# davidesantangelo/krep

Measured on NVIDIA H100. Metric: GB/s scanned (HBM-resident corpus), higher is better.
Workload: dtype u8

## Files before the change

krep_b200/csrc/common.h:

```cpp
#pragma once
#include <cuda_runtime.h>
#include <stdint.h>
#include <stddef.h>
#include <string>
#include <vector>
#include "../../include/krep_b200.h"

namespace kb {

static constexpr int LIT_TAG_BITS = 3;
static constexpr int AC_END_SHIFT = 24;
static constexpr int AC_LEN_SHIFT = 14;
static constexpr uint32_t AC_MAX_PATTERNS = 1u << 14;

enum FilterKind : int
{
    FILTER_ALIGNED4 = 0,
    FILTER_WINDOW4 = 1,
};

struct LitDevParams
{
    const uint8_t *text;
    uint64_t avail_len;
    uint64_t own_begin, own_end;
    uint64_t global_offset;
    int32_t prev_byte, next_byte;
    uint64_t group_begin, group_end;
    uint64_t tail_start;
    uint32_t m;
    uint32_t emit_len;
    uint32_t K[4];
    uint32_t fold;
    uint32_t win_mask;
    uint32_t mulc[3];
    const uint8_t *pat_val;
    const uint8_t *pat_mask;
    uint64_t *out;
    uint64_t cap;
    unsigned long long *counter;
    uint32_t whole_word;
    uint32_t want_positions;
};

struct AcDevTables;
struct AcHostTables;

static constexpr int MAX_DEV = 16;

struct PlanDev
{
    bool ready = false;
    uint8_t *d_pat_val = nullptr, *d_pat_mask = nullptr;
    AcDevTables *ac = nullptr;
};

struct Plan
{
    int algo = 0;
    bool is_ac = false;
    std::string pattern;
    bool case_sensitive = true;
    uint32_t m = 0, emit_len = 0;
    FilterKind filter = FILTER_ALIGNED4;
    uint32_t K[4] = {0, 0, 0, 0};
    uint32_t fold = 0xFFFFFFFFu, win_mask = 0xFFFFFFFFu;
    uint32_t whole_word = 0;
    std::vector<uint8_t> h_val, h_msk;
    bool border_free = true;
    bool built_only_matching = false;
    bool count_lines = false;
    std::vector<std::string> patterns;
    std::vector<uint32_t> pat_lens;
    uint32_t min_len = 0, max_len = 0;
    AcHostTables *ach = nullptr;
    std::string filter_name;
    PlanDev dev[MAX_DEV];
    uint64_t magic = 0x6b7265705f623230ull;
};

struct DevCtx;
void set_error(int code, const char *fmt, ...);
void clear_error();

struct ScanOut
{
    uint64_t count = 0, stored = 0;
    const uint64_t *d_keys = nullptr;
    int overflow = 0;
    const uint64_t *d_bounds = nullptr;
    const uint64_t *h_sorted = nullptr;
    int device = 0;
    uint64_t serial = 0;
};

static constexpr uint64_t LB_SAME_AS_PREV = ~0ull;
static constexpr uint64_t LB_SAME_AS_NEXT = ~0ull - 1;
static constexpr uint64_t LB_OUTSIDE_SHARD = ~0ull - 2;

int launch_scan(DevCtx &C, const Plan *plan, const krep_b200_shard_t *sh, int want_positions, cudaStream_t stream, int slot = 0);
void launch_literal(const Plan *plan, const LitDevParams &p, int sm_count, cudaStream_t s);
int ac_build_tables(Plan *plan);
void ac_free_tables(Plan *plan);
AcDevTables *ac_upload_tables(const Plan *plan);
void ac_free_device(AcDevTables *T);
struct AcLaunch
{
    const uint8_t *text;
    uint64_t avail_len, own_begin, own_end, global_offset;
    int32_t prev_byte, next_byte;
    uint64_t *out;
    uint64_t cap;
    unsigned long long *counter;
    uint32_t whole_word, want_positions;
};
void launch_ac(const Plan *plan, const AcDevTables *T, const AcLaunch &a, int sm_count, cudaStream_t s);
void count_launch(int n = 1);

struct Replay
{
    const uint64_t *keys;
    size_t n;
    const char *text;
    size_t text_len;
    uint64_t base;
    const uint64_t *bounds = nullptr;
};
uint64_t replay_literal(int algo, const search_params_t *P, bool only_matching, uint32_t m,
                        const Replay &r, match_result_t *res);
uint64_t replay_ac(const search_params_t *P, const Replay &r, match_result_t *res);
bool result_push(match_result_t *r, size_t s, size_t e);

static inline unsigned char lower_c(unsigned char c) { return (c >= 'A' && c <= 'Z') ? (unsigned char)(c + 32) : c; }
static inline bool is_alpha_c(unsigned char c) { return (c >= 'A' && c <= 'Z') || (c >= 'a' && c <= 'z'); }
static inline bool is_word_c(int c)
{
    return (c >= '0' && c <= '9') || (c >= 'A' && c <= 'Z') || (c >= 'a' && c <= 'z') || c == '_';
}

}
```

krep_b200/csrc/engine.cu:

```cuda
#include <cub/device/device_radix_sort.cuh>
#include <algorithm>
#include <chrono>
#include <cstdarg>
#include <cstdio>
#include <cstdlib>
#include <cstring>
#include <mutex>
#include <thread>
#include "common.h"
#include "corpus.h"
#include "engine.h"

namespace kb {

static thread_local int t_err = 0;
static thread_local char t_errmsg[512] = "";

void set_error(int code, const char *fmt, ...)
{
    t_err = code;
    va_list ap;
    va_start(ap, fmt);
    vsnprintf(t_errmsg, sizeof t_errmsg, fmt, ap);
    va_end(ap);
    fprintf(stderr, "krep: %s\n", t_errmsg);
}
void clear_error()
{
    t_err = 0;
    t_errmsg[0] = 0;
}

#define CK(call)                                                                                   \
    do                                                                                             \
    {                                                                                              \
        cudaError_t e_ = (call);                                                                   \
        if (e_ != cudaSuccess)                                                                     \
        {                                                                                          \
            set_error(-2, "CUDA error %s at %s:%d (%s)", cudaGetErrorName(e_), __FILE__, __LINE__, \
                      cudaGetErrorString(e_));                                                     \
            return -2;                                                                             \
        }                                                                                          \
    } while (0)

static DevCtx g_ctx[MAX_DEV];
static std::recursive_mutex g_mu;
static std::mutex g_ctx_mu;
static int g_primary = -1;
static int g_visible = -1;
static bool g_keep_visible = false;
static uint64_t g_launches = 0;
static thread_local float t_kernel_ms = 0.f;
static const std::chrono::steady_clock::time_point g_t0 = std::chrono::steady_clock::now();

std::recursive_mutex &engine_mutex() { return g_mu; }
void count_launch(int n) { __atomic_fetch_add(&g_launches, (uint64_t)n, __ATOMIC_RELAXED); }
void add_kernel_ms(float ms) { t_kernel_ms += ms; }
void reset_kernel_ms() { t_kernel_ms = 0.f; }
float get_kernel_ms() { return t_kernel_ms; }
void set_kernel_ms(float ms) { t_kernel_ms = ms; }
void get_error(ErrState *e)
{
    e->code = t_err;
    memcpy(e->msg, t_errmsg, sizeof e->msg);
}
void adopt_error(const ErrState &e)
{
    t_err = e.code;
    memcpy(t_errmsg, e.msg, sizeof t_errmsg);
}

void trace(const char *fmt, ...)
{
    static const bool on = getenv("KREP_B200_TRACE") != nullptr;
    if (!on) return;
    char buf[400];
    va_list ap;
    va_start(ap, fmt);
    vsnprintf(buf, sizeof buf, fmt, ap);
    va_end(ap);
    const double ms = std::chrono::duration<double, std::milli>(std::chrono::steady_clock::now() - g_t0).count();
    fprintf(stderr, "[krep_b200 +%.1f ms] %s\n", ms, buf);
}

static std::thread *g_warm = nullptr;
static std::mutex g_warm_mu;
void warm_join()
{
    std::lock_guard<std::mutex> lk(g_warm_mu);
    if (g_warm && g_warm->joinable() && g_warm->get_id() != std::this_thread::get_id()) g_warm->join();
}
bool warm_running()
{
    std::lock_guard<std::mutex> lk(g_warm_mu);
    return g_warm && g_warm->joinable();
}
static void warm_start()
{
    std::lock_guard<std::mutex> lk(g_warm_mu);
    if (g_warm || g_visible >= 0) return;
    g_warm = new std::thread([] {
        trace("warm-up thread: start");
        if (visible_devices() > 0)
            if (DevCtx *C = ctx_primary()) prewarm_host_path(*C);
        trace("warm-up thread: done");
    });
}
__attribute__((destructor)) static void warm_at_exit()
{
    warm_join();
    trace("library destructor (process exit)");
}

void keep_devices_visible() { g_keep_visible = true; }

int visible_devices()
{
    if (g_visible >= 0) return g_visible;
    static std::mutex mu;
    std::lock_guard<std::mutex> lk(mu);
    if (g_visible >= 0) return g_visible;
    if (!g_keep_visible && !getenv("KREP_B200_KEEP_VISIBLE"))
    {
        const char *v = getenv("KREP_B200_DEVICES");
        const int k = v && atoi(v) > 0 ? atoi(v) : 1;
        std::string list;
        if (const char *cur = getenv("CUDA_VISIBLE_DEVICES"))
        {
            int taken = 0;
            for (const char *q = cur; *q && taken < k;)
            {
                const char *e = strchr(q, ',');
                const size_t len = e ? (size_t)(e - q) : strlen(q);
                if (len)
                {
                    list += (taken ? "," : "") + std::string(q, len);
                    taken++;
                }
                q += len + (e ? 1 : 0);
            }
        }
        else
            for (int d = 0; d < k && d < MAX_DEV; d++) list += (d ? "," : "") + std::to_string(d);
        if (!list.empty())
        {
            setenv("CUDA_VISIBLE_DEVICES", list.c_str(), 1);
            trace("CUDA_VISIBLE_DEVICES=%s", list.c_str());
        }
    }
    int n = 0;
    trace("cudaGetDeviceCount ...");
    cudaError_t e = cudaGetDeviceCount(&n);
    if (e != cudaSuccess)
    {
        cudaGetLastError();
        n = 0;
    }
    trace("cudaGetDeviceCount -> %d", n);
    g_visible = n > MAX_DEV ? MAX_DEV : n;
    return g_visible;
}

int primary_device()
{
    if (g_primary >= 0) return g_primary;
    if (visible_devices() == 0)
    {
        set_error(-1, "no CUDA device available; this engine has no CPU fallback");
        return -1;
    }
    int d = 0;
    if (cudaGetDevice(&d) != cudaSuccess) d = 0;
    g_primary = d;
    return d;
}

static int ctx_create(DevCtx &E, int device)
{
    trace("device %d: creating context", device);
    CK(cudaSetDevice(device));
    cudaDeviceProp prop;
    CK(cudaGetDeviceProperties(&prop, device));
    if (prop.major != 9 || prop.minor != 0)
    {
        set_error(-1, "device %d (%s, sm_%d%d) is not an sm_90 part; kernels are built for sm_90a only", device,
                  prop.name, prop.major, prop.minor);
        return -1;
    }
    E.device = device;
    E.sm_count = prop.multiProcessorCount;
    CK(cudaStreamCreateWithFlags(&E.scan_stream, cudaStreamNonBlocking));
    CK(cudaStreamCreateWithFlags(&E.copy_stream, cudaStreamNonBlocking));
    CK(cudaStreamCreateWithFlags(&E.fin_stream, cudaStreamNonBlocking));
    CK(cudaMalloc(&E.d_counter, 64 * SCAN_SLOTS));
    CK(cudaMemset(E.d_counter, 0, 64 * SCAN_SLOTS));
    CK(cudaEventCreate(&E.ev_ca));
    CK(cudaEventCreate(&E.ev_cb));
    for (int s = 0; s < SCAN_SLOTS; s++)
    {
        CK(cudaMalloc(&E.d_pack[s], (PACK_KEYS + 1) * sizeof(uint64_t)));
        CK(cudaHostAlloc(&E.h_pack[s], (PACK_KEYS + 1) * sizeof(uint64_t), cudaHostAllocMapped | cudaHostAllocPortable));
        E.h_pack[s][0] = 0;
        CK(cudaEventCreate(&E.ev_a[s]));
        CK(cudaEventCreate(&E.ev_b[s]));
        CK(cudaEventCreateWithFlags(&E.ev_done[s], cudaEventDisableTiming));
        CK(cudaEventCreateWithFlags(&E.ev_scanned[s], cudaEventDisableTiming));
        E.counter_clean[s] = true;
    }
    E.ready = true;
    trace("device %d: context ready (%s, %d SMs)", device, prop.name, E.sm_count);
    return 0;
}

DevCtx *ctx_get(int device)
{
    if (device < 0 || device >= MAX_DEV || device >= visible_devices())
    {
        set_error(-1, visible_devices() == 0 ? "no CUDA device available; this engine has no CPU fallback"
                                               : "CUDA device %d is not visible to this process",
                  device);
        return nullptr;
    }
    DevCtx &E = g_ctx[device];
    if (E.ready)
    {
        cudaSetDevice(device);
        return &E;
    }
    static std::mutex mu[MAX_DEV];
    std::lock_guard<std::mutex> lk(mu[device]);
    if (!E.ready && ctx_create(E, device) != 0) return nullptr;
    return &E;
}

DevCtx *ctx_primary()
{
    const int d = primary_device();
    return d < 0 ? nullptr : ctx_get(d);
}

static std::vector<Plan *> g_all_plans;
static std::mutex g_plans_mu;

static void ctx_destroy(DevCtx &E)
{
    if (!E.ready) return;
    cudaSetDevice(E.device);
    cudaDeviceSynchronize();
    for (int s = 0; s < SCAN_SLOTS; s++) cudaFree(E.d_list[s]);
    cudaFree(E.d_alt);
    cudaFree(E.d_sort_tmp);
    cudaFree(E.d_bounds);
    cudaFreeHost(E.h_bounds);
    cudaFreeHost(E.h_batch);
    cudaFree(E.d_counter);
    cudaFree(E.d_ring);
    cudaFree(E.d_line_recs);
    cudaFree(E.d_line_out);
    cudaFreeHost(E.h_line_out);
    cudaFreeHost(E.h_keys);
    for (int s = 0; s < SCAN_SLOTS; s++)
    {
        cudaFree(E.d_pack[s]);
        cudaFreeHost(E.h_pack[s]);
        cudaEventDestroy(E.ev_a[s]);
        cudaEventDestroy(E.ev_b[s]);
        cudaEventDestroy(E.ev_done[s]);
        cudaEventDestroy(E.ev_scanned[s]);
    }
    for (auto &s : E.stage) cudaFreeHost(s.buf);
    for (auto &s : E.stage)
        if (s.ev) cudaEventDestroy(s.ev);
    for (auto ev : E.ev_pool) cudaEventDestroy(ev);
    for (auto ev : E.ring_landed) cudaEventDestroy(ev);
    for (auto ev : E.ring_scanned) cudaEventDestroy(ev);
    cudaEventDestroy(E.ev_ca);
    cudaEventDestroy(E.ev_cb);
    cudaStreamDestroy(E.scan_stream);
    cudaStreamDestroy(E.copy_stream);
    cudaStreamDestroy(E.fin_stream);
    E = DevCtx();
}

void plan_cache_clear();

void engine_shutdown()
{
    std::lock_guard<std::recursive_mutex> lk(g_mu);
    DeviceGuard guard;
    plan_cache_clear();
    {
        std::lock_guard<std::mutex> lp(g_plans_mu);
        for (Plan *p : g_all_plans)
            for (int d = 0; d < MAX_DEV; d++)
            {
                PlanDev &pd = p->dev[d];
                if (!pd.ready) continue;
                cudaSetDevice(d);
                cudaFree(pd.d_pat_val);
                cudaFree(pd.d_pat_mask);
                if (pd.ac) ac_free_device(pd.ac);
                pd = PlanDev();
            }
    }
    for (int d = 0; d < MAX_DEV; d++) ctx_destroy(g_ctx[d]);
    g_primary = -1;
}

int ensure_keys(DevCtx &E, uint64_t cap)
{
    if (cap <= E.key_cap) return 0;
    uint64_t ncap = E.key_cap ? E.key_cap : (1ull << 20);
    while (ncap < cap) ncap *= 2;
    CK(cudaDeviceSynchronize());
    for (int s = 0; s < SCAN_SLOTS; s++)
    {
        cudaFree(E.d_list[s]);
        E.d_list[s] = nullptr;
    }
    cudaFree(E.d_alt);
    E.d_alt = nullptr;
    E.key_cap = 0;
    for (int s = 0; s < SCAN_SLOTS; s++) CK(cudaMalloc(&E.d_list[s], ncap * sizeof(uint64_t)));
    CK(cudaMalloc(&E.d_alt, ncap * sizeof(uint64_t)));
    E.key_cap = ncap;
    return 0;
}

unsigned long long *slot_counter(DevCtx &E, int slot) { return E.d_counter + 8 * slot; }

static uint32_t le32(const uint8_t *b, uint32_t n)
{
    uint32_t v = 0;
    for (uint32_t k = 0; k < n && k < 4; k++) v |= (uint32_t)b[k] << (8 * k);
    return v;
}

void plan_free(Plan *p)
{
    if (!p) return;
    {
        std::lock_guard<std::mutex> lp(g_plans_mu);
        for (size_t i = 0; i < g_all_plans.size(); i++)
            if (g_all_plans[i] == p)
            {
                g_all_plans.erase(g_all_plans.begin() + i);
                break;
            }
    }
    DeviceGuard guard;
    for (int d = 0; d < MAX_DEV; d++)
    {
        PlanDev &pd = p->dev[d];
        if (!pd.ready) continue;
        cudaSetDevice(d);
        cudaFree(pd.d_pat_val);
        cudaFree(pd.d_pat_mask);
        if (pd.ac) ac_free_device(pd.ac);
    }
    if (p->ach) ac_free_tables(p);
    p->magic = 0;
    delete p;
}

const PlanDev *plan_on_device(const Plan *plan, DevCtx &C)
{
    static std::mutex mu;
    PlanDev &pd = const_cast<Plan *>(plan)->dev[C.device];
    if (pd.ready) return &pd;
    std::lock_guard<std::mutex> lk(mu);
    if (pd.ready) return &pd;
    cudaSetDevice(C.device);
    if (plan->is_ac)
    {
        pd.ac = ac_upload_tables(plan);
        if (!pd.ac) return nullptr;
    }
    else
    {
        const size_t m = plan->h_val.size();
        if (cudaMalloc(&pd.d_pat_val, m) != cudaSuccess || cudaMalloc(&pd.d_pat_mask, m) != cudaSuccess ||
            cudaMemcpy(pd.d_pat_val, plan->h_val.data(), m, cudaMemcpyHostToDevice) != cudaSuccess ||
            cudaMemcpy(pd.d_pat_mask, plan->h_msk.data(), m, cudaMemcpyHostToDevice) != cudaSuccess)
        {
            set_error(-2, "CUDA allocation failed while uploading the pattern to device %d", C.device);
            cudaFree(pd.d_pat_val);
            cudaFree(pd.d_pat_mask);
            pd = PlanDev();
            return nullptr;
        }
    }
    pd.ready = true;
    return &pd;
}

static bool border_free(const std::string &s, bool cs)
{
    const size_t m = s.size();
    if (m < 2) return true;
    std::vector<int> pi(m, 0);
    auto ch = [&](size_t i) { return cs ? (unsigned char)s[i] : lower_c((unsigned char)s[i]); };
    for (size_t i = 1; i < m; i++)
    {
        int k = pi[i - 1];
        while (k > 0 && ch(i) != ch((size_t)k)) k = pi[(size_t)k - 1];
        if (ch(i) == ch((size_t)k)) k++;
        pi[i] = k;
    }
    return pi[m - 1] == 0;
}

Plan *plan_build(const search_params_t *P, int algo, bool only_matching)
{
    if (!P) return nullptr;
    Plan *pl = new Plan();
    pl->algo = algo;
    pl->case_sensitive = P->case_sensitive;
    pl->count_lines = P->count_lines_mode;
    if (algo == KREP_B200_ALGO_AC)
    {
        pl->is_ac = true;
        if (P->num_patterns > AC_MAX_PATTERNS)
        {
            set_error(-3, "too many patterns (%zu > %u)", (size_t)P->num_patterns, AC_MAX_PATTERNS);
            delete pl;
            return nullptr;
        }
        for (size_t k = 0; k < P->num_patterns; k++)
        {
            const size_t len = P->pattern_lens[k];
            if (len > 1024)
            {
                set_error(-3, "pattern %zu longer than 1024 bytes (krep.c:77)", k);
                delete pl;
                return nullptr;
            }
            pl->patterns.emplace_back(P->patterns[k] ? P->patterns[k] : "", len);
            pl->pat_lens.push_back((uint32_t)len);
        }
        pl->whole_word = P->whole_word ? 1 : 0;
        if (ac_build_tables(pl) != 0)
        {
            delete pl;
            return nullptr;
        }
        std::lock_guard<std::mutex> lp(g_plans_mu);
        g_all_plans.push_back(pl);
        return pl;
    }
    size_t m = P->pattern_len;
    if (algo == KREP_B200_ALGO_MEMCHR) m = m ? 1 : 0;
    if (m == 0 || m > 1024 || !P->pattern)
    {
        set_error(-3, "literal plan needs 1..1024 pattern bytes (got %zu)", m);
        delete pl;
        return nullptr;
    }
    pl->pattern.assign(P->pattern, m);
    pl->m = (uint32_t)m;
    pl->emit_len = (algo == KREP_B200_ALGO_MEMCHR_SHORT && only_matching) ? 1u : (uint32_t)m;
    pl->border_free = border_free(pl->pattern, pl->case_sensitive);
    pl->built_only_matching = only_matching;
    if (P->whole_word)
    {
        bool tag = pl->emit_len != pl->m;
        if (algo == KREP_B200_ALGO_AVX2 || algo == KREP_B200_ALGO_AVX512 || algo == KREP_B200_ALGO_NEON) tag = true;
        if (!tag && !pl->border_free)
            tag = algo == KREP_B200_ALGO_KMP || (algo == KREP_B200_ALGO_SSE42 && !only_matching);
        pl->whole_word = tag ? 2 : 1;
    }
    pl->h_val.resize(m);
    pl->h_msk.resize(m);
    const uint8_t *pb = (const uint8_t *)pl->pattern.data();
    for (size_t k = 0; k < m; k++)
    {
        pl->h_msk[k] = (!pl->case_sensitive && is_alpha_c(pb[k])) ? 0xDF : 0xFF;
        pl->h_val[k] = pb[k] & pl->h_msk[k];
    }
    pl->fold = pl->case_sensitive ? 0xFFFFFFFFu : 0xDFDFDFDFu;
    if (pl->emit_len >= 7)
    {
        pl->filter = FILTER_ALIGNED4;
        for (int d = 0; d < 4; d++) pl->K[d] = le32(pb + d, 4) & pl->fold;
        pl->win_mask = 0xFFFFFFFFu;
        pl->filter_name = pl->case_sensitive ? "aligned4" : "aligned4-fold";
    }
    else
    {
        pl->filter = FILTER_WINDOW4;
        const uint32_t wl = pl->emit_len < 4 ? pl->emit_len : 4;
        pl->win_mask = wl == 4 ? 0xFFFFFFFFu : ((1u << (8 * wl)) - 1);
        pl->K[0] = le32(pb, wl) & pl->fold & pl->win_mask;
        pl->filter_name = pl->case_sensitive ? "window4" : "window4-fold";
    }
    std::lock_guard<std::mutex> lp(g_plans_mu);
    g_all_plans.push_back(pl);
    return pl;
}

int launch_scan(DevCtx &E, const Plan *plan, const krep_b200_shard_t *sh, int want_positions, cudaStream_t stream, int slot)
{
    if (((uintptr_t)sh->d_text & 15) != 0)
    {
        set_error(-3, "shard text pointer must be 16-byte aligned");
        return -3;
    }
    const PlanDev *pd = plan_on_device(plan, E);
    if (!pd) return -2;
    uint64_t own_end = sh->own_end < sh->avail_len ? sh->own_end : sh->avail_len;
    if (plan->is_ac)
    {
        if (sh->global_offset + sh->avail_len >= (1ull << 40))
        {
            set_error(-3, "pattern-set shards must end below 2^40 bytes of global offset (key layout, csrc/common.h)");
            return -3;
        }
        AcLaunch a;
        a.text = (const uint8_t *)sh->d_text;
        a.avail_len = sh->avail_len;
        a.own_begin = sh->own_begin;
        a.own_end = own_end;
        a.global_offset = sh->global_offset;
        a.prev_byte = sh->prev_byte;
        a.next_byte = sh->next_byte;
        a.out = E.d_list[slot];
        a.cap = want_positions ? E.key_cap : 0;
        a.counter = slot_counter(E, slot);
        a.whole_word = plan->whole_word;
        a.want_positions = (uint32_t)want_positions;
        launch_ac(plan, pd->ac, a, E.sm_count, stream);
        return 0;
    }
    LitDevParams p;
    memset(&p, 0, sizeof p);
    p.text = (const uint8_t *)sh->d_text;
    p.avail_len = sh->avail_len;
    p.own_begin = sh->own_begin;
    p.own_end = own_end;
    p.global_offset = sh->global_offset;
    p.prev_byte = sh->prev_byte;
    p.next_byte = sh->next_byte;
    uint64_t total_groups;
    if (plan->filter == FILTER_ALIGNED4)
    {
        total_groups = sh->avail_len / 16;
        p.tail_start = total_groups ? total_groups * 16 - 3 : 0;
    }
    else
    {
        total_groups = sh->avail_len >= 20 ? (sh->avail_len - 20) / 16 + 1 : 0;
        p.tail_start = total_groups * 16;
    }
    p.group_begin = sh->own_begin / 16;
    p.group_end = (own_end + 2) / 16 + 1;
    if (p.group_end > total_groups) p.group_end = total_groups;
    if (p.group_begin > p.group_end) p.group_begin = p.group_end;
    p.m = plan->m;
    p.emit_len = plan->emit_len;
    for (int d = 0; d < 4; d++) p.K[d] = plan->K[d];
    p.fold = plan->fold;
    p.win_mask = plan->win_mask;
    p.mulc[0] = 1u << 24;
    p.mulc[1] = 1u << 16;
    p.mulc[2] = 1u << 8;
    p.pat_val = pd->d_pat_val;
    p.pat_mask = pd->d_pat_mask;
    p.out = E.d_list[slot];
    p.cap = want_positions ? E.key_cap : 0;
    p.counter = slot_counter(E, slot);
    p.whole_word = plan->whole_word;
    p.want_positions = (uint32_t)want_positions;
    launch_literal(plan, p, E.sm_count, stream);
    return 0;
}

int reset_counter(DevCtx &E, int slot, cudaStream_t stream)
{
    if (E.counter_clean[slot]) return 0;
    CK(cudaMemsetAsync(slot_counter(E, slot), 0, 64, stream));
    E.counter_clean[slot] = true;
    return 0;
}

static constexpr int FIN_THREADS = 512, FIN_SLICES = 16, FIN_KEYS = FIN_THREADS / FIN_SLICES, FIN_PIECE = 2048;

__global__ void __launch_bounds__(FIN_THREADS) k_finish(unsigned long long *counter, const uint64_t *__restrict__ keys, uint64_t cap,
                                                        uint64_t *d_pack, int want_sort)
{
    __shared__ uint64_t s_keys[FIN_PIECE];
    __shared__ unsigned long long s_cnt;
    if (threadIdx.x == 0) s_cnt = counter[0];
    __syncthreads();
    const unsigned long long cnt = s_cnt;
    if (blockIdx.x == 0 && threadIdx.x == 0) d_pack[0] = cnt;
    const bool sorting = want_sort && cnt != 0 && cnt <= PACK_KEYS && cnt <= cap;
    const uint32_t n = sorting ? (uint32_t)cnt : 0u;
    const uint32_t idx = blockIdx.x * FIN_KEYS + threadIdx.x / FIN_SLICES, slice = threadIdx.x % FIN_SLICES;
    if (blockIdx.x * FIN_KEYS < n)
    {
        const uint64_t mine = idx < n ? keys[idx] : ~0ull;
        uint32_t rank = 0;
        for (uint32_t base = 0; base < n; base += FIN_PIECE)
        {
            const uint32_t m = n - base < FIN_PIECE ? n - base : FIN_PIECE;
            for (uint32_t j = threadIdx.x; j < FIN_PIECE; j += FIN_THREADS) s_keys[j] = j < m ? keys[base + j] : ~0ull;
            __syncthreads();
            const uint32_t mr = (m + 63u) & ~63u;
#pragma unroll 8
            for (uint32_t j = slice; j < mr; j += FIN_SLICES) rank += s_keys[j] < mine ? 1u : 0u;
            __syncthreads();
        }
#pragma unroll
        for (int o = 1; o < FIN_SLICES; o <<= 1) rank += __shfl_xor_sync(0xffffffffu, rank, o);
        if (idx < n && slice == 0) d_pack[1 + rank] = mine;
    }
    __syncthreads();
    if (threadIdx.x == 0)
    {
        __threadfence();
        const unsigned long long done = atomicAdd(&counter[1], 1ULL);
        if (done == gridDim.x - 1)
        {
            counter[0] = 0;
            counter[1] = 0;
        }
    }
}

int finish_scan(DevCtx &E, int slot, int want_sort, cudaStream_t stream)
{
    k_finish<<<PACK_KEYS / FIN_KEYS, FIN_THREADS, 0, stream>>>(slot_counter(E, slot), E.d_list[slot], E.key_cap, E.d_pack[slot],
                                                                 (want_sort && E.d_list[slot]) ? 1 : 0);
    CK(cudaGetLastError());
    CK(cudaMemcpyAsync(E.h_pack[slot], E.d_pack[slot], (want_sort ? PACK_KEYS + 1 : 1) * sizeof(uint64_t), cudaMemcpyDeviceToHost, stream));
    CK(cudaEventRecord(E.ev_done[slot], stream));
    count_launch();
    E.counter_clean[slot] = true;
    return 0;
}

int sort_keys(DevCtx &E, int slot, uint64_t n, int end_bit, cudaStream_t stream, const uint64_t **sorted)
{
    *sorted = E.d_list[slot];
    if (n < 2) return 0;
    cub::DoubleBuffer<uint64_t> db(E.d_list[slot], E.d_alt);
    size_t need = 0;
    CK(cub::DeviceRadixSort::SortKeys(nullptr, need, db, (int64_t)n, 0, end_bit, stream));
    if (need > E.sort_tmp_bytes)
    {
        CK(cudaStreamSynchronize(stream));
        cudaFree(E.d_sort_tmp);
        E.d_sort_tmp = nullptr;
        E.sort_tmp_bytes = 0;
        CK(cudaMalloc(&E.d_sort_tmp, need));
        E.sort_tmp_bytes = need;
    }
    CK(cub::DeviceRadixSort::SortKeys(E.d_sort_tmp, need, db, (int64_t)n, 0, end_bit, stream));
    *sorted = db.Current();
    return 0;
}

static int bits_for(uint64_t v)
{
    int b = 1;
    while (b < 64 && (v >> b)) b++;
    return b;
}

int key_end_bit(const Plan *plan, uint64_t max_offset)
{
    const int shift = plan->is_ac ? AC_END_SHIFT : LIT_TAG_BITS;
    int b = bits_for(max_offset) + shift;
    return b > 64 ? 64 : b;
}

__global__ void __launch_bounds__(256) k_line_bounds(const uint8_t *__restrict__ text, uint64_t avail, uint64_t go,
                                                     const uint64_t *__restrict__ keys, uint64_t n, int is_ac, int has_prev,
                                                     int has_next, uint64_t *__restrict__ out)
{
    const uint64_t i = ((uint64_t)blockIdx.x * blockDim.x + threadIdx.x) >> 5;
    const int lane = threadIdx.x & 31;
    if (i >= n) return;
    auto start_of = [&](uint64_t key) -> uint64_t {
        if (!is_ac) return (key >> LIT_TAG_BITS) - go;
        return (key >> AC_END_SHIFT) - (1024 - ((key >> AC_LEN_SHIFT) & 1023)) - go;
    };
    const uint64_t s = start_of(keys[i]);
    const uint64_t lb = (!is_ac && i > 0) ? start_of(keys[i - 1]) : 0;
    const uint64_t ub = (!is_ac && i + 1 < n) ? start_of(keys[i + 1]) : avail;
    uint64_t ls = (!is_ac && i > 0) ? LB_SAME_AS_PREV : (has_prev ? LB_OUTSIDE_SHARD : go);
    for (uint64_t hi = s; hi > lb;)
    {
        const uint64_t w0 = hi >= lb + 128 ? hi - 128 : lb;
        int best = -1;
#pragma unroll
        for (int k = 0; k < 4; k++)
        {
            const uint64_t p = w0 + (uint64_t)lane * 4 + k;
            if (p < hi && text[p] == '\n') best = lane * 4 + k;
        }
        best = __reduce_max_sync(0xffffffffu, best);
        if (best >= 0)
        {
            ls = go + w0 + (uint64_t)best + 1;
            break;
        }
        hi = w0;
    }
    uint64_t le = (!is_ac && i + 1 < n) ? LB_SAME_AS_NEXT : (has_next ? LB_OUTSIDE_SHARD : go + avail);
    for (uint64_t lo = s; lo < ub; lo += 128)
    {
        int best = 1 << 20;
#pragma unroll
        for (int k = 3; k >= 0; k--)
        {
            const uint64_t p = lo + (uint64_t)lane * 4 + k;
            if (p < ub && text[p] == '\n') best = lane * 4 + k;
        }
        best = __reduce_min_sync(0xffffffffu, best);
        if (best < (1 << 20))
        {
            le = go + lo + (uint64_t)best;
            break;
        }
    }
    if (lane == 0)
    {
        out[2 * i] = ls;
        out[2 * i + 1] = le;
    }
}

static int line_bounds(DevCtx &E, const Plan *plan, const krep_b200_shard_t *sh, const uint64_t *d_sorted, uint64_t n,
                       cudaStream_t stream, const uint64_t **d_bounds)
{
    *d_bounds = nullptr;
    if (n == 0) return 0;
    if (2 * n > E.bounds_cap)
    {
        CK(cudaStreamSynchronize(stream));
        cudaFree(E.d_bounds);
        E.d_bounds = nullptr;
        E.bounds_cap = 0;
        const uint64_t cap = 2 * n + n / 4 + 1024;
        CK(cudaMalloc(&E.d_bounds, cap * sizeof(uint64_t)));
        E.bounds_cap = cap;
    }
    const uint64_t threads = n * 32;
    const int has_prev = sh->prev_byte >= 0 && sh->prev_byte != '\n';
    const int has_next = sh->next_byte >= 0 && sh->next_byte != '\n';
    k_line_bounds<<<(unsigned)((threads + 255) / 256), 256, 0, stream>>>((const uint8_t *)sh->d_text, sh->avail_len, sh->global_offset,
                                                                        d_sorted, n, plan->is_ac ? 1 : 0, has_prev, has_next, E.d_bounds);
    CK(cudaGetLastError());
    count_launch();
    *d_bounds = E.d_bounds;
    return 0;
}

int scan_begin(DevCtx &E, const Plan *plan, const krep_b200_shard_t *sh, int want_positions, cudaStream_t stream, int *slot_out)
{
    if (!stream) stream = E.scan_stream;
    if (want_positions && ensure_keys(E, 1) != 0) return -2;
    const int slot = E.next_slot;
    if (E.pend[slot].active)
    {
        set_error(-3, "krep_b200_scan_shard_begin: %d scans are already in flight on device %d", SCAN_SLOTS, E.device);
        return -3;
    }
    CK(cudaStreamWaitEvent(stream, E.ev_done[slot], 0));
    if (reset_counter(E, slot, stream) != 0) return -2;
    CK(cudaEventRecord(E.ev_a[slot], stream));
    int rc = launch_scan(E, plan, sh, want_positions, stream, slot);
    if (rc != 0) return rc;
    CK(cudaEventRecord(E.ev_b[slot], stream));
    CK(cudaGetLastError());
    if (finish_scan(E, slot, want_positions, stream) != 0) return -2;
    PendingScan &P = E.pend[slot];
    P.active = true;
    P.plan = plan;
    P.shard = *sh;
    P.want_positions = want_positions;
    P.stream = stream;
    E.next_slot = (slot + 1) % SCAN_SLOTS;
    *slot_out = slot;
    return 0;
}

int scan_end(DevCtx &E, int slot, ScanOut *out)
{
    PendingScan &P = E.pend[slot];
    if (slot < 0 || slot >= SCAN_SLOTS || !P.active)
    {
        set_error(-3, "krep_b200_scan_shard_end: no scan in flight in slot %d", slot);
        return -3;
    }
    P.active = false;
    const Plan *plan = P.plan;
    const krep_b200_shard_t *sh = &P.shard;
    cudaStream_t stream = P.stream;
    reset_kernel_ms();
    for (int attempt = 0; attempt < 3; attempt++)
    {
        CK(cudaEventSynchronize(E.ev_done[slot]));
        const uint64_t cnt = E.h_pack[slot][0];
        float ms = 0.f;
        cudaEventElapsedTime(&ms, E.ev_a[slot], E.ev_b[slot]);
        add_kernel_ms(ms);
        *out = ScanOut();
        out->count = cnt;
        out->device = E.device;
        out->serial = ++E.serial;
        E.result_stream = stream;
        if (!P.want_positions) return 0;
        if (cnt <= E.key_cap)
        {
            int rc = 0;
            out->stored = cnt;
            if (cnt <= PACK_KEYS)
            {
                out->d_keys = E.d_pack[slot] + 1;
                out->h_sorted = E.h_pack[slot] + 1;
            }
            else
                rc = sort_keys(E, slot, cnt, key_end_bit(plan, sh->global_offset + sh->avail_len), stream, &out->d_keys);
            if (rc == 0 && plan->count_lines) rc = line_bounds(E, plan, sh, out->d_keys, cnt, stream, &out->d_bounds);
            return rc;
        }
        out->overflow = 1;
        for (int s2 = 0; s2 < SCAN_SLOTS; s2++)
            if (s2 != slot && E.pend[s2].active)
            {
                set_error(-3, "krep_b200_scan_shard_end: the occurrence list overflowed while another scan is in flight; end each "
                              "scan before beginning the next until the list has grown");
                return -3;
            }
        if (ensure_keys(E, cnt + cnt / 8 + 1024) != 0) return -2;
        if (reset_counter(E, slot, stream) != 0) return -2;
        CK(cudaEventRecord(E.ev_a[slot], stream));
        int rc = launch_scan(E, plan, sh, 1, stream, slot);
        if (rc != 0) return rc;
        CK(cudaEventRecord(E.ev_b[slot], stream));
        if (finish_scan(E, slot, 1, stream) != 0) return -2;
    }
    set_error(-4, "occurrence list kept overflowing");
    return -4;
}

int scan_shard(DevCtx &E, const Plan *plan, const krep_b200_shard_t *sh, int want_positions, cudaStream_t stream, ScanOut *out)
{
    int slot = 0;
    int rc = scan_begin(E, plan, sh, want_positions, stream, &slot);
    if (rc != 0) return rc;
    return scan_end(E, slot, out);
}

int fetch_keys(DevCtx &E, const ScanOut &so, const uint64_t **h)
{
    *h = nullptr;
    if (so.stored == 0) return 0;
    if (so.h_sorted)
    {
        *h = so.h_sorted;
        return 0;
    }
    if (so.stored > E.h_keys_cap)
    {
        cudaFreeHost(E.h_keys);
        E.h_keys = nullptr;
        E.h_keys_cap = 0;
        uint64_t cap = so.stored + so.stored / 4;
        if (cap < (1u << 16)) cap = 1u << 16;
        CK(cudaMallocHost(&E.h_keys, cap * sizeof(uint64_t)));
        E.h_keys_cap = cap;
    }
    cudaStream_t s = E.result_stream ? E.result_stream : E.scan_stream;
    CK(cudaMemcpyAsync(E.h_keys, so.d_keys, so.stored * sizeof(uint64_t), cudaMemcpyDeviceToHost, s));
    CK(cudaStreamSynchronize(s));
    *h = E.h_keys;
    return 0;
}

uint64_t merge_key_lists(const uint64_t *const *lists, const uint64_t *counts, uint32_t n_lists, uint64_t *dst)
{
    uint64_t total = 0;
    std::vector<uint64_t> cut;
    for (uint32_t i = 0; i < n_lists; i++)
    {
        if (counts[i] == 0) continue;
        if (dst + total != lists[i]) memmove(dst + total, lists[i], counts[i] * sizeof(uint64_t));
        cut.push_back(total);
        total += counts[i];
    }
    for (size_t i = 1; i < cut.size(); i++)
        if (dst[cut[i] - 1] > dst[cut[i]]) std::inplace_merge(dst, dst + cut[i], dst + (i + 1 < cut.size() ? cut[i + 1] : total));
    return total;
}

__global__ void __launch_bounds__(256) k_corpus(const __grid_constant__ CorpusParams c, uint8_t *dst, uint64_t global_offset,
                                                uint64_t len)
{
    const uint64_t groups = (len + 15) / 16;
    for (uint64_t g = (uint64_t)blockIdx.x * blockDim.x + threadIdx.x; g < groups; g += (uint64_t)gridDim.x * blockDim.x)
    {
        alignas(16) uint8_t b[16];
        corpus_fill16(c, global_offset + g * 16, b);
        const uint64_t off = g * 16;
        if (off + 16 <= len && (((uintptr_t)(dst + off)) & 15) == 0)
            *reinterpret_cast<uint4 *>(dst + off) = *reinterpret_cast<const uint4 *>(b);
        else
            for (int k = 0; k < 16 && off + k < len; k++) dst[off + k] = b[k];
    }
}

static int corpus_params(const krep_b200_corpus_spec_t *spec, CorpusParams *c)
{
    memset(c, 0, sizeof *c);
    c->seed = spec->seed;
    c->plant_seed = spec->plant_seed;
    c->plant_period = spec->plant_period;
    c->needle_len = spec->needle_len;
    c->flags = spec->flags;
    if (spec->needle_len > 64)
    {
        set_error(-3, "corpus needle longer than 64 bytes");
        return -3;
    }
    if (spec->plant_period && (spec->plant_period % 16 != 0 || spec->plant_period < 4ull * spec->needle_len + 32))
    {
        set_error(-3, "corpus plant_period must be a multiple of 16 and >= 4*needle_len+32");
        return -3;
    }
    if (spec->needle_len) memcpy(c->needle, spec->needle, spec->needle_len);
    return 0;
}

}

using namespace kb;
// ... 256 lines not shown
```

krep_b200/csrc/engine.h:

```cpp
#pragma once
#include <mutex>
#include <vector>
#include "common.h"

namespace kb {

static constexpr uint32_t PACK_KEYS = 16384;
static constexpr int SCAN_SLOTS = 2;

struct StageSlot
{
    uint8_t *buf = nullptr;
    cudaEvent_t ev = nullptr;
    bool in_flight = false;
};

struct PendingScan
{
    bool active = false;
    const Plan *plan = nullptr;
    krep_b200_shard_t shard;
    int want_positions = 0;
    cudaStream_t stream = nullptr;
};

struct DevCtx
{
    bool ready = false;
    int device = 0, sm_count = 0;
    cudaStream_t scan_stream = nullptr, copy_stream = nullptr;
    cudaStream_t fin_stream = nullptr;
    unsigned long long *d_counter = nullptr;
    bool counter_clean[SCAN_SLOTS] = {false, false};
    uint64_t *d_list[SCAN_SLOTS] = {nullptr, nullptr};
    uint64_t *d_alt = nullptr;
    uint64_t key_cap = 0;
    void *d_sort_tmp = nullptr;
    size_t sort_tmp_bytes = 0;
    uint64_t *d_bounds = nullptr;
    uint64_t bounds_cap = 0;
    uint64_t *h_bounds = nullptr;
    uint64_t h_bounds_cap = 0;
    uint64_t *d_pack[SCAN_SLOTS] = {nullptr, nullptr}, *h_pack[SCAN_SLOTS] = {nullptr, nullptr};
    cudaEvent_t ev_a[SCAN_SLOTS] = {nullptr, nullptr}, ev_b[SCAN_SLOTS] = {nullptr, nullptr};
    cudaEvent_t ev_done[SCAN_SLOTS] = {nullptr, nullptr};
    cudaEvent_t ev_scanned[SCAN_SLOTS] = {nullptr, nullptr};
    cudaEvent_t ev_ca = nullptr, ev_cb = nullptr;
    PendingScan pend[SCAN_SLOTS];
    int next_slot = 0;
    uint64_t serial = 0;
    cudaStream_t result_stream = nullptr;
    void *d_line_recs = nullptr;
    uint64_t line_recs_cap = 0;
    uint64_t *d_line_out = nullptr, *h_line_out = nullptr;
    uint64_t line_out_cap = 0;
    uint8_t *d_ring = nullptr;
    size_t ring_slot_bytes = 0;
    int ring_slots = 0;
    std::vector<cudaEvent_t> ring_landed, ring_scanned;
    std::vector<StageSlot> stage;
    size_t stage_bytes = 0;
    std::vector<cudaEvent_t> ev_pool;
    uint64_t *h_keys = nullptr;
    uint64_t h_keys_cap = 0;
    uint8_t *h_batch = nullptr;
    uint64_t h_batch_cap = 0;
};

struct ErrState
{
    int code = 0;
    char msg[512] = "";
};
void get_error(ErrState *e);
void adopt_error(const ErrState &e);

std::recursive_mutex &engine_mutex();
int primary_device();
int visible_devices();
DevCtx *ctx_get(int device);
DevCtx *ctx_primary();
void engine_shutdown();
void prewarm_host_path(DevCtx &C);
void keep_devices_visible();
void warm_join();
bool warm_running();

struct DeviceGuard
{
    int saved = -1;
    DeviceGuard() { if (cudaGetDevice(&saved) != cudaSuccess) { saved = -1; cudaGetLastError(); } }
    ~DeviceGuard() { if (saved >= 0) cudaSetDevice(saved); }
};

Plan *plan_build(const search_params_t *P, int algo, bool only_matching);
void plan_free(Plan *p);
const PlanDev *plan_on_device(const Plan *p, DevCtx &C);
int resolve_algo(const search_params_t *P, int algo);

unsigned long long *slot_counter(DevCtx &C, int slot);
int scan_begin(DevCtx &C, const Plan *plan, const krep_b200_shard_t *sh, int want_positions, cudaStream_t stream, int *slot);
int scan_end(DevCtx &C, int slot, ScanOut *out);
int scan_shard(DevCtx &C, const Plan *plan, const krep_b200_shard_t *sh, int want_positions, cudaStream_t stream, ScanOut *out);
int finish_scan(DevCtx &C, int slot, int want_sort, cudaStream_t stream);
int ensure_keys(DevCtx &C, uint64_t cap);
int reset_counter(DevCtx &C, int slot, cudaStream_t stream);
int sort_keys(DevCtx &C, int slot, uint64_t n, int end_bit, cudaStream_t stream, const uint64_t **sorted);
int key_end_bit(const Plan *plan, uint64_t max_offset);
int fetch_keys(DevCtx &C, const ScanOut &so, const uint64_t **h);
void add_kernel_ms(float ms);
void reset_kernel_ms();
float get_kernel_ms();
void set_kernel_ms(float ms);
void trace(const char *fmt, ...);

bool count_lines_eligible(const Plan *plan, const search_params_t *P, int algo);
int ensure_line_out(DevCtx &C, uint64_t n);
int launch_count_lines(DevCtx &C, const Plan *plan, const krep_b200_shard_t *sh, cudaStream_t stream, uint64_t index);
uint64_t combine_line_records(const uint64_t *recs, size_t n);

uint64_t merge_key_lists(const uint64_t *const *lists, const uint64_t *counts, uint32_t n_lists, uint64_t *dst);

}
```

krep_b200/csrc/scan_literal.cu:

```cuda
#include <mutex>
#include "common.h"
#include "lit_filters.cuh"

#ifndef KREP_B200_WARP_EMIT
#define KREP_B200_WARP_EMIT 1
#endif

namespace kb {

__device__ __noinline__ unsigned verify_emit(const LitDevParams &p, long long cand)
{
    const unsigned tag = verify_exact(p, cand);
    if (!tag) return 0;
    if (p.want_positions)
    {
        const unsigned long long slot = atomicAdd(p.counter, 1ULL);
        if (slot < p.cap) p.out[slot] = ((p.global_offset + (uint64_t)cand) << LIT_TAG_BITS) | (tag & 7u);
        return 0;
    }
    return 1;
}

__device__ __noinline__ unsigned slow_aligned4(const LitDevParams &p, uint64_t group, uint4 v)
{
    unsigned n = 0;
    const uint32_t w[4] = {v.x & p.fold, v.y & p.fold, v.z & p.fold, v.w & p.fold};
#pragma unroll
    for (int k = 0; k < 4; k++)
#pragma unroll
        for (int d = 0; d < 4; d++)
            if (w[k] == p.K[d]) n += verify_emit(p, (long long)(group * 16 + 4 * k) - d);
    return n;
}

template <bool WINDOW>
__device__ __noinline__ unsigned emit_warp(const LitDevParams &p, uint64_t group, uint4 v, uint32_t nx, bool mine)
{
    const uint32_t lane = threadIdx.x & 31;
    uint32_t valid = 0;
    uint64_t tags = 0;
    if (mine)
    {
        const uint32_t w[5] = {v.x, v.y, v.z, v.w, nx};
        if (WINDOW)
        {
            const uint32_t mask = p.fold & p.win_mask, k0 = p.K[0];
#pragma unroll
            for (int k = 0; k < 4; k++)
#pragma unroll
                for (int r = 0; r < 4; r++)
                {
                    const uint32_t win = r == 0 ? w[k] : __funnelshift_r(w[k], w[k + 1], 8 * r);
                    if ((win & mask) == k0)
                    {
                        const unsigned t = verify_exact(p, (long long)(group * 16 + 4 * k + r));
                        if (t)
                        {
                            valid |= 1u << (4 * k + r);
                            tags |= (uint64_t)(t & 7u) << (3 * (4 * k + r));
                        }
                    }
                }
        }
        else
        {
#pragma unroll
            for (int k = 0; k < 4; k++)
#pragma unroll
                for (int d = 0; d < 4; d++)
                    if ((w[k] & p.fold) == p.K[d])
                    {
                        const unsigned t = verify_exact(p, (long long)(group * 16 + 4 * k) - d);
                        if (t)
                        {
                            valid |= 1u << (4 * k + d);
                            tags |= (uint64_t)(t & 7u) << (3 * (4 * k + d));
                        }
                    }
        }
    }
    const uint32_t n = (uint32_t)__popc(valid);
    if (!p.want_positions) return n;
    uint32_t incl = n;
#pragma unroll
    for (int o = 1; o < 32; o <<= 1)
    {
        const uint32_t t = __shfl_up_sync(0xffffffffu, incl, o);
        if (lane >= (uint32_t)o) incl += t;
    }
    const uint32_t total = __shfl_sync(0xffffffffu, incl, 31);
    if (total == 0) return 0;
    unsigned long long base = 0;
    if (lane == 31) base = atomicAdd(p.counter, (unsigned long long)total);
    base = __shfl_sync(0xffffffffu, base, 31);
    unsigned long long slot = base + (incl - n);
    while (valid)
    {
        const uint32_t i = (uint32_t)__ffs(valid) - 1;
        valid &= valid - 1;
        const long long start = WINDOW ? (long long)(group * 16 + i) : (long long)(group * 16 + (i & ~3u)) - (long long)(i & 3u);
        if (slot < p.cap) p.out[slot] = ((p.global_offset + (uint64_t)start) << LIT_TAG_BITS) | ((tags >> (3 * i)) & 7u);
        slot++;
    }
    return 0;
}

__device__ __forceinline__ void tail_and_count(const LitDevParams &p, unsigned long long local_cnt)
{
    if (blockIdx.x == 0 && threadIdx.x < 32 && p.avail_len >= p.emit_len)
    {
        const uint64_t last = p.avail_len - p.emit_len;
        for (uint64_t s = p.tail_start + threadIdx.x; s <= last; s += 32) local_cnt += verify_emit(p, (long long)s);
    }
    if (!p.want_positions)
    {
#pragma unroll
        for (int o = 16; o > 0; o >>= 1) local_cnt += __shfl_xor_sync(0xffffffffu, local_cnt, o);
        if ((threadIdx.x & 31) == 0 && local_cnt) atomicAdd(p.counter, local_cnt);
    }
}

template <bool FOLD, int UNROLL>
__global__ void __launch_bounds__(256, 4) k_lit_aligned4(const __grid_constant__ LitDevParams p)
{
    const uint4 *__restrict__ t4 = reinterpret_cast<const uint4 *>(p.text);
    const uint32_t k0 = p.K[0], k1 = p.K[1], k2 = p.K[2], k3 = p.K[3], fold = p.fold;
    unsigned long long local_cnt = 0;
    const uint64_t tile = (uint64_t)blockDim.x * UNROLL;
    const uint64_t stride = (uint64_t)gridDim.x * tile;
    uint64_t g0 = p.group_begin + (uint64_t)blockIdx.x * tile;
    for (; g0 + tile <= p.group_end; g0 += stride)
    {
        uint4 v[UNROLL];
#pragma unroll
        for (int u = 0; u < UNROLL; u++) v[u] = ld_stream(t4 + g0 + (uint64_t)u * blockDim.x + threadIdx.x);
        bool hit = false;
#pragma unroll
        for (int u = 0; u < UNROLL; u++) hit |= hit_vec<FOLD>(v[u], fold, k0, k1, k2, k3);
#if KREP_B200_WARP_EMIT
        if (__any_sync(0xffffffffu, hit))
        {
#pragma unroll
            for (int u = 0; u < UNROLL; u++)
            {
                const bool mine = hit_vec<FOLD>(v[u], fold, k0, k1, k2, k3);
                if (__any_sync(0xffffffffu, mine))
                    local_cnt += emit_warp<false>(p, g0 + (uint64_t)u * blockDim.x + threadIdx.x, v[u], 0u, mine);
            }
        }
#else
        if (hit)
        {
#pragma unroll
            for (int u = 0; u < UNROLL; u++)
                if (hit_vec<FOLD>(v[u], fold, k0, k1, k2, k3))
                    local_cnt += slow_aligned4(p, g0 + (uint64_t)u * blockDim.x + threadIdx.x, v[u]);
        }
#endif
    }
    if (g0 < p.group_end)
    {
        for (int u = 0; u < UNROLL; u++)
        {
            const uint64_t g = g0 + (uint64_t)u * blockDim.x + threadIdx.x;
            if (g < p.group_end)
            {
                const uint4 v = ld_stream(t4 + g);
                if (hit_vec<FOLD>(v, fold, k0, k1, k2, k3)) local_cnt += slow_aligned4(p, g, v);
            }
        }
    }
    tail_and_count(p, local_cnt);
}

__device__ __noinline__ unsigned slow_window4(const LitDevParams &p, uint64_t group, uint4 v, uint32_t nx)
{
    unsigned n = 0;
    const uint32_t w[5] = {v.x, v.y, v.z, v.w, nx};
    const uint32_t mask = p.fold & p.win_mask, k0 = p.K[0];
#pragma unroll
    for (int k = 0; k < 4; k++)
#pragma unroll
        for (int r = 0; r < 4; r++)
        {
            const uint32_t win = r == 0 ? w[k] : __funnelshift_r(w[k], w[k + 1], 8 * r);
            if ((win & mask) == k0) n += verify_emit(p, (long long)(group * 16 + 4 * k + r));
        }
    return n;
}

#ifndef KREP_B200_W4_NX
#define KREP_B200_W4_NX 2
#endif
#ifndef KREP_B200_W4_WARP_EMIT
#define KREP_B200_W4_WARP_EMIT 0
#endif
#ifdef KREP_B200_W4_CS
#define WLOAD(q) ld_stream(q)
#else
#define WLOAD(q) __ldg(q)
#endif
template <bool FOLD, bool MASKED, int UNROLL>
__global__ void __launch_bounds__(256, 4) k_lit_window4(const __grid_constant__ LitDevParams p)
{
    const uint4 *__restrict__ t4 = reinterpret_cast<const uint4 *>(p.text);
    const uint32_t fold = p.fold, mask = p.win_mask, k0 = p.K[0];
    const uint32_t c1 = p.mulc[0], c2 = p.mulc[1], c3 = p.mulc[2];
    const bool lane31 = (threadIdx.x & 31) == 31;
    unsigned long long local_cnt = 0;
    const uint64_t tile = (uint64_t)blockDim.x * UNROLL;
    const uint64_t stride = (uint64_t)gridDim.x * tile;
    uint64_t g0 = p.group_begin + (uint64_t)blockIdx.x * tile;
    for (; g0 + tile <= p.group_end; g0 += stride)
    {
        uint4 v[UNROLL];
        uint32_t nx[UNROLL];
#pragma unroll
        for (int u = 0; u < UNROLL; u++)
        {
            const uint4 *q = t4 + g0 + (uint64_t)u * blockDim.x + threadIdx.x;
            v[u] = WLOAD(q);
#if KREP_B200_W4_NX == 0
            nx[u] = __ldg(reinterpret_cast<const uint32_t *>(q + 1));
#elif KREP_B200_W4_NX == 2
            nx[u] = 0u;
            asm volatile("{\n\t.reg .pred p;\n\tsetp.ne.u32 p, %2, 0;\n\t@p ld.global.nc.u32 %0, [%1];\n\t}"
                         : "+r"(nx[u])
                         : "l"(reinterpret_cast<const uint32_t *>(q + 1)), "r"((uint32_t)lane31));
#else
            nx[u] = lane31 ? __ldg(reinterpret_cast<const uint32_t *>(q + 1)) : 0u;
#endif
        }
#if KREP_B200_W4_NX != 0
#pragma unroll
        for (int u = 0; u < UNROLL; u++)
        {
            const uint32_t nb = __shfl_down_sync(0xffffffffu, v[u].x, 1);
#if KREP_B200_W4_NX == 2
            nx[u] = lane31 ? nx[u] : nb;
#else
            if (!lane31) nx[u] = nb;
#endif
        }
#endif
        uint32_t hm = 0;
#pragma unroll
        for (int u = 0; u < UNROLL; u++)
            hm |= hit_vec_w<FOLD, MASKED>(v[u], nx[u], fold, mask, k0, c1, c2, c3) ? (1u << u) : 0u;
        if constexpr (MASKED || KREP_B200_W4_WARP_EMIT)
        {
            const uint32_t anyhm = __reduce_or_sync(0xffffffffu, hm);
            if (anyhm)
            {
#pragma unroll
                for (int u = 0; u < UNROLL; u++)
                    if ((anyhm >> u) & 1u)
                        local_cnt += emit_warp<true>(p, g0 + (uint64_t)u * blockDim.x + threadIdx.x, v[u], nx[u], (hm >> u) & 1u);
            }
        }
        else if (hm)
        {
#pragma unroll
            for (int u = 0; u < UNROLL; u++)
                if ((hm >> u) & 1u) local_cnt += slow_window4(p, g0 + (uint64_t)u * blockDim.x + threadIdx.x, v[u], nx[u]);
        }
    }
    if (g0 < p.group_end)
    {
        for (int u = 0; u < UNROLL; u++)
        {
            const uint64_t g = g0 + (uint64_t)u * blockDim.x + threadIdx.x;
            if (g < p.group_end)
            {
                const uint4 v = ld_stream(t4 + g);
                const uint32_t nx = __ldg(reinterpret_cast<const uint32_t *>(t4 + g + 1));
                if (hit_vec_w<FOLD, MASKED>(v, nx, fold, mask, k0, c1, c2, c3)) local_cnt += slow_window4(p, g, v, nx);
            }
        }
    }
    tail_and_count(p, local_cnt);
}

static int g_occ[6] = {0, 0, 0, 0, 0, 0};

template <typename K>
static int occupancy(K kernel)
{
    int nb = 0;
    cudaOccupancyMaxActiveBlocksPerMultiprocessor(&nb, kernel, 256, 0);
    return nb > 0 ? nb : 1;
}

void launch_literal(const Plan *plan, const LitDevParams &p, int sm_count, cudaStream_t s)
{
    constexpr int UNROLL = 4;
    static std::once_flag once;
    std::call_once(once, [] {
        g_occ[0] = occupancy(k_lit_aligned4<false, UNROLL>);
        g_occ[1] = occupancy(k_lit_aligned4<true, UNROLL>);
        g_occ[2] = occupancy(k_lit_window4<false, false, UNROLL>);
        g_occ[3] = occupancy(k_lit_window4<true, false, UNROLL>);
        g_occ[4] = occupancy(k_lit_window4<false, true, UNROLL>);
        g_occ[5] = occupancy(k_lit_window4<true, true, UNROLL>);
    });
    const uint64_t groups = p.group_end > p.group_begin ? p.group_end - p.group_begin : 0;
    const uint64_t tile = 256ull * UNROLL;
    uint64_t tiles = (groups + tile - 1) / tile;
    if (tiles == 0) tiles = 1;
    const bool folded = plan->fold != 0xFFFFFFFFu, masked = plan->win_mask != 0xFFFFFFFFu;
    const int which = plan->filter == FILTER_WINDOW4 ? 2 + (folded ? 1 : 0) + (masked ? 2 : 0) : (folded ? 1 : 0);
    uint64_t resident = (uint64_t)sm_count * g_occ[which];
    const unsigned grid = (unsigned)(tiles < resident ? tiles : resident);
    if (which == 2)
        k_lit_window4<false, false, UNROLL><<<grid, 256, 0, s>>>(p);
    else if (which == 3)
        k_lit_window4<true, false, UNROLL><<<grid, 256, 0, s>>>(p);
    else if (which == 4)
        k_lit_window4<false, true, UNROLL><<<grid, 256, 0, s>>>(p);
    else if (which == 5)
        k_lit_window4<true, true, UNROLL><<<grid, 256, 0, s>>>(p);
    else if (which == 1)
        k_lit_aligned4<true, UNROLL><<<grid, 256, 0, s>>>(p);
    else
        k_lit_aligned4<false, UNROLL><<<grid, 256, 0, s>>>(p);
    count_launch();
}

}
```

Before: 3122.

## Run finish kernel on high-priority stream beside literal scan with reserved SM room

For literal scans that are not masked and own at most 16 GiB, the scan grid drops one resident block per SM. The finish/sort kernel then runs on a high-priority stream after an event, using a grid-stride loop over an SM-count grid, so it can overlap the next scan. A shared-memory carveout preference is set for both kernels so they can co-reside, and k_finish gets a min-blocks launch bound. This trades some scan occupancy for overlap of the finish step, and adds cross-stream event dependencies.

Result: faster. 3161 (median of 6 runs) (+1.2%).

```diff
diff --git a/krep_b200/csrc/common.h b/krep_b200/csrc/common.h
--- a/krep_b200/csrc/common.h
+++ b/krep_b200/csrc/common.h
@@ -99,7 +99,9 @@
 static constexpr uint64_t LB_OUTSIDE_SHARD = ~0ull - 2;
 
 int launch_scan(DevCtx &C, const Plan *plan, const krep_b200_shard_t *sh, int want_positions, cudaStream_t stream, int slot = 0);
-void launch_literal(const Plan *plan, const LitDevParams &p, int sm_count, cudaStream_t s);
+void launch_literal(const Plan *plan, const LitDevParams &p, int sm_count, bool leave_room, cudaStream_t s);
+bool literal_leaves_room(const Plan *plan, uint64_t owned_bytes);
+cudaError_t literal_set_carveout(int percent);
 int ac_build_tables(Plan *plan);
 void ac_free_tables(Plan *plan);
 AcDevTables *ac_upload_tables(const Plan *plan);
diff --git a/krep_b200/csrc/engine.cu b/krep_b200/csrc/engine.cu
--- a/krep_b200/csrc/engine.cu
+++ b/krep_b200/csrc/engine.cu
@@ -175,6 +175,8 @@
     return d;
 }
 
+static cudaError_t set_finish_carveout();
+
 static int ctx_create(DevCtx &E, int device)
 {
     trace("device %d: creating context", device);
@@ -191,7 +193,10 @@
     E.sm_count = prop.multiProcessorCount;
     CK(cudaStreamCreateWithFlags(&E.scan_stream, cudaStreamNonBlocking));
     CK(cudaStreamCreateWithFlags(&E.copy_stream, cudaStreamNonBlocking));
-    CK(cudaStreamCreateWithFlags(&E.fin_stream, cudaStreamNonBlocking));
+    int least_prio = 0, greatest_prio = 0;
+    CK(cudaDeviceGetStreamPriorityRange(&least_prio, &greatest_prio));
+    CK(cudaStreamCreateWithPriority(&E.fin_stream, cudaStreamNonBlocking, greatest_prio));
+    CK(set_finish_carveout());
     CK(cudaMalloc(&E.d_counter, 64 * SCAN_SLOTS));
     CK(cudaMemset(E.d_counter, 0, 64 * SCAN_SLOTS));
     CK(cudaEventCreate(&E.ev_ca));
@@ -528,6 +533,7 @@
         a.counter = slot_counter(E, slot);
         a.whole_word = plan->whole_word;
         a.want_positions = (uint32_t)want_positions;
+        E.fin_beside[slot] = false;
         launch_ac(plan, pd->ac, a, E.sm_count, stream);
         return 0;
     }
@@ -570,7 +576,8 @@
     p.counter = slot_counter(E, slot);
     p.whole_word = plan->whole_word;
     p.want_positions = (uint32_t)want_positions;
-    launch_literal(plan, p, E.sm_count, stream);
+    E.fin_beside[slot] = literal_leaves_room(plan, own_end - sh->own_begin);
+    launch_literal(plan, p, E.sm_count, E.fin_beside[slot], stream);
     return 0;
 }
 
@@ -584,8 +591,8 @@
 
 static constexpr int FIN_THREADS = 512, FIN_SLICES = 16, FIN_KEYS = FIN_THREADS / FIN_SLICES, FIN_PIECE = 2048;
 
-__global__ void __launch_bounds__(FIN_THREADS) k_finish(unsigned long long *counter, const uint64_t *__restrict__ keys, uint64_t cap,
-                                                        uint64_t *d_pack, int want_sort)
+__global__ void __launch_bounds__(FIN_THREADS, 4) k_finish(unsigned long long *counter, const uint64_t *__restrict__ keys, uint64_t cap,
+                                                           uint64_t *d_pack, int want_sort)
 {
     __shared__ uint64_t s_keys[FIN_PIECE];
     __shared__ unsigned long long s_cnt;
@@ -595,9 +602,10 @@
     if (blockIdx.x == 0 && threadIdx.x == 0) d_pack[0] = cnt;
     const bool sorting = want_sort && cnt != 0 && cnt <= PACK_KEYS && cnt <= cap;
     const uint32_t n = sorting ? (uint32_t)cnt : 0u;
-    const uint32_t idx = blockIdx.x * FIN_KEYS + threadIdx.x / FIN_SLICES, slice = threadIdx.x % FIN_SLICES;
-    if (blockIdx.x * FIN_KEYS < n)
-    {
+    const uint32_t slice = threadIdx.x % FIN_SLICES;
+    for (uint32_t group = blockIdx.x; group * FIN_KEYS < n; group += gridDim.x)
+    {
+        const uint32_t idx = group * FIN_KEYS + threadIdx.x / FIN_SLICES;
         const uint64_t mine = idx < n ? keys[idx] : ~0ull;
         uint32_t rank = 0;
         for (uint32_t base = 0; base < n; base += FIN_PIECE)
@@ -627,13 +635,30 @@
     }
 }
 
+static constexpr int FIN_CARVEOUT_PCT = 40;
+
+static cudaError_t set_finish_carveout()
+{
+    const cudaError_t e = cudaFuncSetAttribute(k_finish, cudaFuncAttributePreferredSharedMemoryCarveout, FIN_CARVEOUT_PCT);
+    return e != cudaSuccess ? e : literal_set_carveout(FIN_CARVEOUT_PCT);
+}
+
 int finish_scan(DevCtx &E, int slot, int want_sort, cudaStream_t stream)
 {
-    k_finish<<<PACK_KEYS / FIN_KEYS, FIN_THREADS, 0, stream>>>(slot_counter(E, slot), E.d_list[slot], E.key_cap, E.d_pack[slot],
-                                                                 (want_sort && E.d_list[slot]) ? 1 : 0);
+    const bool beside = E.fin_beside[slot];
+    cudaStream_t fs = stream;
+    if (beside)
+    {
+        CK(cudaEventRecord(E.ev_scanned[slot], stream));
+        CK(cudaStreamWaitEvent(E.fin_stream, E.ev_scanned[slot], 0));
+        fs = E.fin_stream;
+    }
+    const unsigned grid = beside ? (unsigned)E.sm_count : PACK_KEYS / FIN_KEYS;
+    k_finish<<<grid, FIN_THREADS, 0, fs>>>(slot_counter(E, slot), E.d_list[slot], E.key_cap, E.d_pack[slot],
+                                          (want_sort && E.d_list[slot]) ? 1 : 0);
     CK(cudaGetLastError());
-    CK(cudaMemcpyAsync(E.h_pack[slot], E.d_pack[slot], (want_sort ? PACK_KEYS + 1 : 1) * sizeof(uint64_t), cudaMemcpyDeviceToHost, stream));
-    CK(cudaEventRecord(E.ev_done[slot], stream));
+    CK(cudaMemcpyAsync(E.h_pack[slot], E.d_pack[slot], (want_sort ? PACK_KEYS + 1 : 1) * sizeof(uint64_t), cudaMemcpyDeviceToHost, fs));
+    CK(cudaEventRecord(E.ev_done[slot], fs));
     count_launch();
     E.counter_clean[slot] = true;
     return 0;
diff --git a/krep_b200/csrc/engine.h b/krep_b200/csrc/engine.h
--- a/krep_b200/csrc/engine.h
+++ b/krep_b200/csrc/engine.h
@@ -30,6 +30,7 @@
     int device = 0, sm_count = 0;
     cudaStream_t scan_stream = nullptr, copy_stream = nullptr;
     cudaStream_t fin_stream = nullptr;
+    bool fin_beside[SCAN_SLOTS] = {false, false};
     unsigned long long *d_counter = nullptr;
     bool counter_clean[SCAN_SLOTS] = {false, false};
     uint64_t *d_list[SCAN_SLOTS] = {nullptr, nullptr};
diff --git a/krep_b200/csrc/scan_literal.cu b/krep_b200/csrc/scan_literal.cu
--- a/krep_b200/csrc/scan_literal.cu
+++ b/krep_b200/csrc/scan_literal.cu
@@ -283,46 +283,50 @@
 
 static int g_occ[6] = {0, 0, 0, 0, 0, 0};
 
-template <typename K>
-static int occupancy(K kernel)
-{
-    int nb = 0;
-    cudaOccupancyMaxActiveBlocksPerMultiprocessor(&nb, kernel, 256, 0);
-    return nb > 0 ? nb : 1;
-}
-
-void launch_literal(const Plan *plan, const LitDevParams &p, int sm_count, cudaStream_t s)
-{
-    constexpr int UNROLL = 4;
+static constexpr int LIT_UNROLL = 4;
+using LitKernel = void (*)(LitDevParams);
+static const LitKernel k_lit[6] = {k_lit_aligned4<false, LIT_UNROLL>,        k_lit_aligned4<true, LIT_UNROLL>,
+                                   k_lit_window4<false, false, LIT_UNROLL>, k_lit_window4<true, false, LIT_UNROLL>,
+                                   k_lit_window4<false, true, LIT_UNROLL>,  k_lit_window4<true, true, LIT_UNROLL>};
+
+cudaError_t literal_set_carveout(int percent)
+{
+    for (int k = 0; k < 4; k++)
+    {
+        const cudaError_t e = cudaFuncSetAttribute(k_lit[k], cudaFuncAttributePreferredSharedMemoryCarveout, percent);
+        if (e != cudaSuccess) return e;
+    }
+    return cudaSuccess;
+}
+
+static constexpr uint64_t ROOM_MAX_BYTES = 16ull << 30;
+
+bool literal_leaves_room(const Plan *plan, uint64_t owned_bytes)
+{
+    const bool masked = plan->filter == FILTER_WINDOW4 && plan->win_mask != 0xFFFFFFFFu;
+    return !masked && owned_bytes <= ROOM_MAX_BYTES;
+}
+
+void launch_literal(const Plan *plan, const LitDevParams &p, int sm_count, bool leave_room, cudaStream_t s)
+{
     static std::once_flag once;
     std::call_once(once, [] {
-        g_occ[0] = occupancy(k_lit_aligned4<false, UNROLL>);
-        g_occ[1] = occupancy(k_lit_aligned4<true, UNROLL>);
-        g_occ[2] = occupancy(k_lit_window4<false, false, UNROLL>);
-        g_occ[3] = occupancy(k_lit_window4<true, false, UNROLL>);
-        g_occ[4] = occupancy(k_lit_window4<false, true, UNROLL>);
-        g_occ[5] = occupancy(k_lit_window4<true, true, UNROLL>);
+        for (int k = 0; k < 6; k++)
+        {
+            cudaOccupancyMaxActiveBlocksPerMultiprocessor(&g_occ[k], k_lit[k], 256, 0);
+            if (g_occ[k] < 1) g_occ[k] = 1;
+        }
     });
     const uint64_t groups = p.group_end > p.group_begin ? p.group_end - p.group_begin : 0;
-    const uint64_t tile = 256ull * UNROLL;
+    const uint64_t tile = 256ull * LIT_UNROLL;
     uint64_t tiles = (groups + tile - 1) / tile;
     if (tiles == 0) tiles = 1;
     const bool folded = plan->fold != 0xFFFFFFFFu, masked = plan->win_mask != 0xFFFFFFFFu;
     const int which = plan->filter == FILTER_WINDOW4 ? 2 + (folded ? 1 : 0) + (masked ? 2 : 0) : (folded ? 1 : 0);
-    uint64_t resident = (uint64_t)sm_count * g_occ[which];
+    const int per_sm = leave_room && g_occ[which] > 1 ? g_occ[which] - 1 : g_occ[which];
+    const uint64_t resident = (uint64_t)sm_count * per_sm;
     const unsigned grid = (unsigned)(tiles < resident ? tiles : resident);
-    if (which == 2)
-        k_lit_window4<false, false, UNROLL><<<grid, 256, 0, s>>>(p);
-    else if (which == 3)
-        k_lit_window4<true, false, UNROLL><<<grid, 256, 0, s>>>(p);
-    else if (which == 4)
-        k_lit_window4<false, true, UNROLL><<<grid, 256, 0, s>>>(p);
-    else if (which == 5)
-        k_lit_window4<true, true, UNROLL><<<grid, 256, 0, s>>>(p);
-    else if (which == 1)
-        k_lit_aligned4<true, UNROLL><<<grid, 256, 0, s>>>(p);
-    else
-        k_lit_aligned4<false, UNROLL><<<grid, 256, 0, s>>>(p);
+    k_lit[which]<<<grid, 256, 0, s>>>(p);
     count_launch();
 }
 
```
